# WeGoToMars/indexed_bzip2

Hardware: AMD Instinct MI355X
Metric: decompressed MB/s (whole node), 2 GiB Silesia bz2-9 (higher is better)
Workload: dtype u8

## Files before the change

### indexed_bzip2_amd/csrc/bz2_device.hip

```cpp
#include <hip/hip_runtime.h>

#include <cstdio>
#include <atomic>
#include <chrono>
#include <cstdlib>
#include <algorithm>
#include <cstring>
#include <condition_variable>
#include <memory>
#include <mutex>
#include <string>
#include <thread>
#include <vector>

#include "../../include/mi355x_bz2.h"
#include "bz2_kernels.hip.h"
#include "bz2_stage1.hip.h"
#include "bz2_hscan.hip.h"
#include "bz2_walk.hip.h"
#include "bz2_plan.hpp"
#include "bz2_scratch.hpp"
#include "bz2_lanes.hpp"
#include "bz2_ctx.hpp"

// ... 836 lines not shown
mi355x::decodeBatchBegin( mi355x_bz2_ctx* c, const uint64_t* offsets, const uint64_t* endBytes, uint32_t n )
{
    if ( c == nullptr || ( n > 0 && offsets == nullptr ) ) return MI355X_BZ2_ERR_INVALID_ARGUMENT;
    const std::scoped_lock lock( c->mutex );
    if ( c->pendingBlocks != 0 ) {
        c->lastError = "a batch is already in flight on this context: call mi355x_bz2_decode_batch_end first";
        return MI355X_BZ2_ERR_INVALID_ARGUMENT;
    }
    c->outSize = 0;
    c->lastBlocks = 0;
    if ( n == 0 ) return MI355X_BZ2_OK;
    if ( n > MI355X_BZ2_MAX_BATCH_BLOCKS ) {
        c->lastError = "more than MI355X_BZ2_MAX_BATCH_BLOCKS blocks in one batch: split it";
        return MI355X_BZ2_ERR_INVALID_ARGUMENT;
    }
    if ( c->dIn == nullptr && !c->upload ) {
        c->lastError = "no input set";
        return MI355X_BZ2_ERR_INVALID_ARGUMENT;
    }
    HIP_TRY( c, hipSetDevice( c->device ) );
    const BatchSwitches switches = readSwitches();
    const auto tBegin = std::chrono::steady_clock::now();
    int rc = ensureScratch( c, n );
    if ( rc != MI355X_BZ2_OK ) return rc;
    rc = ensureOutput( c, std::max<uint64_t>( (uint64_t)n * 900000u, c->outSizeHint ) );
    if ( rc != MI355X_BZ2_OK ) return rc;
    const auto tScratch = std::chrono::steady_clock::now();
    const uint8_t* inBase = nullptr;
    uint64_t inSize = 0;
    {
        uint64_t last = 0;
        for ( uint32_t i = 0; i < n; ++i ) last = std::max( last, offsets[i] );
        rc = awaitInput( c, last / 8 + 2400000, &inBase, &inSize );
        if ( rc != MI355X_BZ2_OK ) return rc;
    }
    const auto tInput = std::chrono::steady_clock::now();

    const bool crowd = walkChainOf( c->device ).liveContexts.load() >= 3;
    const uint32_t lanes = lanesNow( c );
    PlanOverrides knobs = switches.plan;
    if ( lanes == 1 ) knobs.noSplit = true;
    c->plan = planBatch( offsets, n, inSize, crowd, knobs );
    c->trace = switches.trace;
    const BatchPlan& plan = c->plan;
    const LaneLayout layout = layLanes( lanes, plan );
    rc = ensureLanes( c, layout );
    if ( rc != MI355X_BZ2_OK ) return rc;
    std::copy( plan.slotOf.begin(), plan.slotOf.end(), c->hSlotOf );
    std::copy( plan.offsets.begin(), plan.offsets.end(), c->hOffsets );
    std::copy( plan.order.begin(), plan.order.end(), c->hOrder );
    if ( endBytes != nullptr ) {
        for ( uint32_t i = 0; i < n; ++i ) c->hEnds[plan.slotOf[i]] = endBytes[i];
    }

    for ( auto& bits : c->launched ) bits = 0;
    if ( c->inPending ) {
        HIP_TRY( c, hipStreamWaitEvent( c->stream, c->inReady, 0 ) );
        c->inPending = false;
    }
    c->inFlight = ( inBase == c->in[0].bytes && inBase != nullptr ) ? 0 : ( ( inBase == c->in[1].bytes && inBase != nullptr ) ? 1 : -1 );
    HIP_TRY( c, hipEventRecord( c->evStep[0], c->stream ) );
    HIP_TRY( c, hipMemcpyAsync( c->dOffsets, c->hOffsets, (size_t)n * sizeof( uint64_t ), hipMemcpyHostToDevice, c->stream ) );
    HIP_TRY( c, hipMemcpyAsync( c->dOrder, c->hOrder, (size_t)n * sizeof( uint32_t ), hipMemcpyHostToDevice, c->stream ) );
    HIP_TRY( c, hipMemcpyAsync( c->dSlotOf, c->hSlotOf, (size_t)n * sizeof( uint32_t ), hipMemcpyHostToDevice, c->stream ) );
    if ( endBytes != nullptr ) {
        HIP_TRY( c, hipMemcpyAsync( c->dEnds, c->hEnds, (size_t)n * sizeof( uint64_t ), hipMemcpyHostToDevice, c->stream ) );
    }
    HIP_TRY( c, hipEventRecord( c->evStep[1], c->stream ) );
    auto streamOfLane = [&] ( int l ) { return l == layout.highLane ? c->highStream : c->lane[l]; };
    auto streamOf = [&] ( int g ) { return streamOfLane( layout.laneOf[g] ); };
    {
        bool waits[MAX_LANES]{};
        for ( int g = 0; g < plan.groups; ++g ) {
            const int l = layout.laneOf[g];
            if ( l != 0 && !waits[l] ) HIP_TRY( c, hipStreamWaitEvent( streamOfLane( l ), c->evStep[1], 0 ) );
            waits[l] = true;
        }
    }
    int lastGroupOfLane[MAX_LANES];
    for ( auto& g : lastGroupOfLane ) g = -1;

    const dim3 walkGrid( WALK_QUEUES * plan.walkWgsPerXcd );
    for ( int launch = 0; launch < plan.groups; ++launch ) {
        const int g = plan.expensive >= 0 ? ( launch == 0 ? plan.expensive : launch - 1 ) : launch;
        const uint32_t m = plan.count[g], first = plan.first[g];
        hipStream_t q = streamOf( g );
        BlockMeta* const meta = c->dMeta + first;
        HuffMeta* const hmeta = c->dHmeta + first;
        uint8_t* const sel = c->dSel + (size_t)first * SEL_STRIDE;
        uint16_t* const sym = c->dSym + (size_t)first * SYM_STRIDE;
        uint8_t* const stb = c->dStb + (size_t)first * 256;
        uint8_t* const lcol = c->dL + (size_t)first * L_STRIDE;
        uint32_t* const tab = c->dTab + (size_t)first * TAB_STRIDE;
        uint8_t* const rbuf = c->dR + (size_t)first * L_STRIDE;
        uint32_t* const segLen = c->dSegLen + (size_t)first * SEG_STRIDE;
        uint32_t* const segSucc = c->dSegSucc + (size_t)first * SEG_STRIDE;
        uint32_t* const segCont = c->dSegCont + (size_t)first * SEG_STRIDE;
        uint2* const chain = c->dChain + (size_t)first * SEG_STRIDE;
        uint32_t* const stash = c->dStash + (size_t)first * SEG_STRIDE * ( STASH_BYTES / 4 );
        const uint32_t* const order = c->dOrder + first;
        WalkPlan* const walkPlan = c->dPlan + g;
        uint32_t* const walkBlk = c->dWalkBlk + (size_t)g * ( c->capacity + 16 );
        uint32_t* const walkPre = c->dWalkPre + (size_t)g * ( c->capacity + 16 );

        {
            ScanMeta* const smeta = c->dSmeta + first;
            HuffTables* const htab = c->dHtab + first;
            uint32_t* const gpos = c->dGpos + (size_t)first * GPOS_STRIDE;
            const auto* const inWords = reinterpret_cast<const uint32_t*>( inBase );
            const uint64_t* const ends = endBytes != nullptr ? c->dEnds + first : nullptr;
            if ( plan.scanWaves[g] == 8 ) {
                TIMED_LAUNCH( c, g, q, 12, k_hscan_spec<8>, dim3( m ), dim3( 512 ), 0, q, inWords, inSize, c->dOffsets + first,
                              ends, meta, hmeta, smeta, sel, stb, htab, gpos, m, order );
            } else if ( plan.scanWaves[g] == 4 ) {
                TIMED_LAUNCH( c, g, q, 12, k_hscan_spec<4>, dim3( m ), dim3( 256 ), 0, q, inWords, inSize, c->dOffsets + first,
                              ends, meta, hmeta, smeta, sel, stb, htab, gpos, m, order );
            } else {
                TIMED_LAUNCH( c, g, q, 12, ( k_hscan<1, REGS_SCAN> ), dim3( m ), dim3( 64 ), sizeof( ScanShared<1> ), q, inWords,
                              inSize, c->dOffsets + first, ends, meta, hmeta, smeta, sel, stb, htab, gpos, m, order );
            }
#define HSYM( T ) TIMED_LAUNCH( c, g, q, 13, k_hsym<T>, dim3( ( MAX_SCAN_GROUPS + ( T ) * SYM_CHUNKS - 1 ) / ( ( T ) * SYM_CHUNKS ), m ), dim3( T ), \
                                sizeof( SymShared<T> ), q, inWords, meta, hmeta, smeta, sel, htab, gpos, sym )
            HSYM( SYM_GROUPS );
#undef HSYM
        }
#define MTF256( STRIDE, STREAM, INDEX ) \
        TIMED_LAUNCH( c, g, STREAM, INDEX, ( k_mtf<STRIDE, MTF_THREADS, REGS_MTF> ), dim3( m ), dim3( MTF_THREADS ), \
                      sizeof( MtfShared<STRIDE, MTF_THREADS> ), STREAM, meta, hmeta, sym, stb, lcol, m, order )
        const hipStream_t side = layout.sideLaneOf[g] >= 0 ? streamOfLane( layout.sideLaneOf[g] ) : q;
        if ( side != q ) {
            HIP_TRY( c, hipEventRecord( c->evFork[g], q ) );
            HIP_TRY( c, hipStreamWaitEvent( side, c->evFork[g], 0 ) );
        }
        if ( plan.mtfSmallLanes == 1024 ) {
            TIMED_LAUNCH( c, g, side, 11, ( k_mtf<MTF_SMALL_STRIDE, 1024> ), dim3( m ), dim3( 1024 ), sizeof( MtfShared<MTF_SMALL_STRIDE, 1024> ), side, meta, hmeta, sym, stb, lcol, m, order );
        } else if ( plan.mtfSmallLanes == 512 ) {
            TIMED_LAUNCH( c, g, side, 11, ( k_mtf<MTF_SMALL_STRIDE, 512> ), dim3( m ), dim3( 512 ), sizeof( MtfShared<MTF_SMALL_STRIDE, 512> ), side, meta, hmeta, sym, stb, lcol, m, order );
        } else {
            MTF256( MTF_SMALL_STRIDE, side, 11 );
        }
        if ( side != q ) HIP_TRY( c, hipEventRecord( c->evJoin[g], side ) );
        if ( plan.mtfSmallLanes > 256 ) {
            TIMED_LAUNCH( c, g, q, 1, ( k_mtf<MTF_LANE_STRIDE, 512> ), dim3( m ), dim3( 512 ), sizeof( MtfShared<MTF_LANE_STRIDE, 512> ), q, meta, hmeta, sym, stb, lcol, m, order );
        } else {
            MTF256( MTF_LANE_STRIDE, q, 1 );
        }
        if ( side != q ) HIP_TRY( c, hipStreamWaitEvent( q, c->evJoin[g], 0 ) );
#undef MTF256
        if ( plan.bwtSlices > 1 ) {
            uint32_t* const counts = c->dBwtCounts + (size_t)first * BWT_COUNTS_PER_BLOCK;
            TIMED( c, g, q, 2, hipLaunchKernelGGL( k_bwt_count, dim3( plan.bwtSlices, m ), dim3( 1024 ), 0, q, meta, lcol, counts, plan.bwtSlices );
                               hipLaunchKernelGGL( k_bwt_rank, dim3( plan.bwtSlices, m ), dim3( 1024 ), 0, q, meta, lcol, tab, counts, plan.bwtSlices ) );
        } else {
            TIMED_LAUNCH( c, g, q, 2, k_bwt_build, dim3( m ), dim3( 1024 ), 0, q, meta, lcol, tab );
        }
        TIMED_LAUNCH( c, g, q, 10, k_walk_plan, dim3( 1 ), dim3( 256 ), 0, q, meta, m, walkPlan, walkBlk, walkPre );
        {
            WalkChain& walks = walkChainOf( c->device );
            const std::scoped_lock walkLock( walks.mutex );
            if ( walks.last != nullptr ) HIP_TRY( c, hipStreamWaitEvent( q, walks.last, 0 ) );
            TIMED_LAUNCH( c, g, q, 3, k_walk, walkGrid, dim3( WALK_THREADS ), 0, q,
                          meta, tab, walkPlan, walkBlk, walkPre, segLen, segSucc, plan.walkChunk, stash, segCont );
            hipEvent_t& slot = walks.events[walks.next++ % 64];
            if ( slot == nullptr ) HIP_TRY( c, hipEventCreateWithFlags( &slot, hipEventDisableTiming ) );
            HIP_TRY( c, hipEventRecord( slot, q ) );
            walks.last = slot;
        }
        TIMED_LAUNCH( c, g, q, 4, k_link2, dim3( m ), dim3( LINK_THREADS ), sizeof( LinkShared ), q, meta, segLen, segSucc, chain );
        TIMED_LAUNCH( c, g, q, 5, k_emit, dim3( ( SEG_STRIDE + EMIT_THREADS * EMIT_TILES - 1 ) / ( EMIT_THREADS * EMIT_TILES ), m ), dim3( EMIT_THREADS ), 0, q,
                      meta, tab, chain, stash, segCont, rbuf );
        static_assert( (size_t)SEG_STRIDE * STASH_BYTES >= L_STRIDE );
        TIMED_LAUNCH( c, g, q, 6, k_replicate, dim3( m ), dim3( 256 ), 0, q, meta, rbuf, reinterpret_cast<uint8_t*>( stash ),
                      (size_t)SEG_STRIDE * STASH_BYTES );
        TIMED_LAUNCH( c, g, q, 7, k_rle<false>, dim3( m ), dim3( RLE_THREADS ), 0, q, meta, rbuf, (uint8_t*)nullptr );
        lastGroupOfLane[layout.laneOf[g]] = g;
    }
    HIP_TRY( c, hipGetLastError() );
    for ( uint32_t l = 1; l < MAX_LANES; ++l ) {
        const int g = lastGroupOfLane[l];
        if ( g < 0 ) continue;
        HIP_TRY( c, hipEventRecord( c->evGroupDone[g], streamOfLane( (int)l ) ) );
        HIP_TRY( c, hipStreamWaitEvent( c->stream, c->evGroupDone[g], 0 ) );
    }

    if ( c->outputHold != nullptr ) {
        HIP_TRY( c, hipStreamWaitEvent( c->stream, c->outputHold, 0 ) );
        c->outputHold = nullptr;
    }
    hipLaunchKernelGGL( k_offsets, dim3( 1 ), dim3( OFFSETS_THREADS ), 0, c->stream, c->dMeta, c->dSlotOf, n,
                        c->out[c->outCurrent].capacity, c->dTotals );
    rc = queueOutput( c, n, c->dTotals + 1 );
    if ( rc != MI355X_BZ2_OK ) return rc;
    HIP_TRY( c, hipMemcpyAsync( c->hTotals, c->dTotals, 2 * sizeof( uint64_t ), hipMemcpyDeviceToHost, c->stream ) );
    c->pendingBlocks = n;
    if ( switches.readerTrace ) {
        const auto ms = [] ( auto a, auto b ) { return std::chrono::duration<double, std::milli>( b - a ).count(); };
        std::fprintf( stderr, "[device] begin of %u blocks: scratch %.1f ms, input %.1f ms, plan + launches %.1f ms\n", n,
                      ms( tBegin, tScratch ), ms( tScratch, tInput ), ms( tInput, std::chrono::steady_clock::now() ) );
    }
    return MI355X_BZ2_OK;
}

int
mi355x::resultBuffer( mi355x_bz2_ctx* c, uint64_t size, uint64_t keep, uint8_t** device )
{
    if ( c == nullptr || device == nullptr ) return MI355X_BZ2_ERR_INVALID_ARGUMENT;
    const std::scoped_lock lock( c->mutex );
    HIP_TRY( c, hipSetDevice( c->device ) );
    GrowBuffer& result = c->result;
    if ( size > result.capacity || result.bytes == nullptr ) {
        HIP_TRY( c, hipStreamSynchronize( c->stream ) );
        const uint64_t cap = std::max<uint64_t>( { size, result.capacity + result.capacity / 2, uint64_t( 1 ) << 20 } );
        if ( c->dOut == result.bytes ) c->dOut = c->out[c->outCurrent].bytes;
        GrowBuffer grown;
        HIP_TRY( c, grown.grow( c, cap, cap, cap ) );
        if ( keep != 0 && result.bytes != nullptr ) {
            HIP_TRY( c, hipMemcpyAsync( grown.bytes, result.bytes, std::min( keep, result.capacity ), hipMemcpyDeviceToDevice, c->stream ) );
            HIP_TRY( c, hipStreamSynchronize( c->stream ) );
        }
        std::swap( result, grown );
        grown.putAside( c, cap );
    }
    *device = result.bytes;
    return MI355X_BZ2_OK;
}

void*&
mi355x::encoderOf( mi355x_bz2_ctx* c, void ( *release )( void* ) )
{
    c->encoderFree = release;
    return c->encoder;
}

int
mi355x::deviceOf( const mi355x_bz2_ctx* c )
{
    return c->device;
}

uint64_t
mi355x::inputCapacity( const mi355x_bz2_ctx* c )
{
    const std::scoped_lock lock( c->mutex );
    return std::max( c->in[0].capacity, c->in[1].capacity );
}

void
mi355x::setLastError( mi355x_bz2_ctx* c, const std::string& message )
{
    const std::scoped_lock lock( c->mutex );
    c->lastError = message;
}

int
mi355x::publishResult( mi355x_bz2_ctx* c, uint64_t size )
{
    if ( c == nullptr || size > c->result.capacity ) return MI355X_BZ2_ERR_INVALID_ARGUMENT;
    const std::scoped_lock lock( c->mutex );
    c->dOut = c->result.bytes;
    c->outSize = size;
    return MI355X_BZ2_OK;
}

extern "C" {

int
mi355x_bz2_decode_batch_end( mi355x_bz2_ctx* c, mi355x_bz2_block_result* results, uint64_t* totalDecoded )
{
    if ( c == nullptr ) return MI355X_BZ2_ERR_INVALID_ARGUMENT;
    const std::scoped_lock lock( c->mutex );
    if ( totalDecoded ) *totalDecoded = 0;
    const uint32_t n = c->pendingBlocks;
    if ( n == 0 ) return MI355X_BZ2_OK;
    if ( results == nullptr ) return MI355X_BZ2_ERR_INVALID_ARGUMENT;
    c->pendingBlocks = 0;
    const BatchPlan& plan = c->plan;
    int rc = MI355X_BZ2_OK;
    HIP_TRY( c, hipSetDevice( c->device ) );
    HIP_TRY( c, hipStreamSynchronize( c->stream ) );
    uint64_t total = c->hTotals[0];
    if ( c->hTotals[1] != 0 ) {
        total = 0;
        for ( uint32_t i = 0; i < n; ++i ) {
            BlockMeta& m = c->hMeta[c->hSlotOf[i]];
            m.out_off = total;
            if ( m.walk_ok ) total += m.decoded_size;
        }
        rc = ensureOutput( c, total );
        if ( rc != MI355X_BZ2_OK ) return rc;
        HIP_TRY( c, hipMemcpyAsync( c->dMeta, c->hMeta, (size_t)n * sizeof( BlockMeta ), hipMemcpyHostToDevice, c->stream ) );
        rc = queueOutput( c, n, nullptr );
        if ( rc != MI355X_BZ2_OK ) return rc;
        HIP_TRY( c, hipStreamSynchronize( c->stream ) );
    }
    c->outSizeHint = std::max( c->outSizeHint, total );

    for ( uint32_t i = 0; i < n; ++i ) {
        const BlockMeta& m = c->hMeta[c->hSlotOf[i]];
        mi355x_bz2_block_result& r = results[i];
        r.encoded_offset_bits = m.enc_off;
        r.encoded_size_bits = ( m.status == ST_OK || m.status == ST_CRC ) ? m.enc_size : 0;
        r.decoded_size = m.status == ST_OK || m.status == ST_CRC ? m.decoded_size : 0;
        r.data_offset = m.out_off;
        r.header_crc = m.header_crc;
        r.computed_crc = m.computed_crc;
        const bool loopDone = m.status == ST_OK || m.status == ST_CRC || m.status == ST_ORIGPTR_DATA;
        r.bwt_length = loopDone ? m.n : 0;
// ... 363 lines not shown
```

### indexed_bzip2_amd/csrc/bz2_kernels.hip.h

```cpp
#pragma once

#include <hip/hip_runtime.h>
#include <stdint.h>

#include "bz2_scratch.hpp"

namespace bz2gpu
{
constexpr uint32_t MAX_N = 900000;
constexpr uint32_t MIN_SEG_STRIDE = 16;
constexpr uint32_t MARK = 0x80000000u;
constexpr uint32_t LF_MASK = 0xFFFFFu;
constexpr uint32_t INVALID_OFF = 0xFFFFFFFFu;

enum Status : int32_t {
    ST_OK = 0, ST_EOF = 1, ST_BAD_MAGIC = 2, ST_RANDOMIZED = 3, ST_ORIGPTR_RANGE = 4, ST_GROUP_COUNT = 5,
    ST_SELECTOR_COUNT = 6, ST_SELECTOR_UNARY = 7, ST_CODE_LENGTH = 8, ST_HUFFMAN_LENGTHS = 9,
    ST_SELECTOR_OVERRUN = 10, ST_INVALID_CODE = 11, ST_RUN_OVERFLOW = 12, ST_DATA_OVERFLOW = 13,
    ST_ORIGPTR_DATA = 14, ST_CRC = 15
};

struct BlockMeta
{
    uint64_t enc_off;
// ... 27 lines not shown
{
    return __builtin_amdgcn_readfirstlane( v );
}

__device__ __forceinline__ uint32_t
be32( uint32_t word )
{
    return __builtin_bswap32( word );
}

__device__ __forceinline__ uint32_t
lane_id()
{
    return threadIdx.x & 63u;
}

struct BitRd
{
    const uint32_t* w;
    uint64_t nwords;
    uint64_t size_bits;
    uint32_t tail_mask;
    uint64_t buf;
    uint32_t n;
    uint64_t widx;
    uint64_t pos;
    bool eof;

    __device__ __forceinline__ uint32_t
    loadw( uint64_t i ) const
    {
        uint32_t v = 0;
        if ( i < nwords ) {
            v = sfl( be32( w[i] ) );
        }
        return v;
    }

    __device__ __forceinline__ void
    init( const uint32_t* words, uint64_t size_bytes, uint64_t bitpos )
    {
        w = words;
        nwords = ( size_bytes + 3 ) >> 2;
        size_bits = size_bytes * 8;
        const uint32_t r = (uint32_t)( size_bytes & 3 );
        tail_mask = r == 0 ? 0xFFFFFFFFu : ( 0xFFFFFFFFu << ( 32 - 8 * r ) );
        pos = bitpos;
        eof = false;
        widx = bitpos >> 5;
        const uint32_t sh = (uint32_t)( bitpos & 31 );
        const uint64_t hi = loadw( widx ), lo = loadw( widx + 1 );
        buf = ( ( hi << 32 ) | lo ) << sh;
        n = 64 - sh;
        widx += 2;
    }

    __device__ __forceinline__ void
    refill()
    {
        if ( n <= 32 ) {
            buf |= (uint64_t)loadw( widx ) << ( 32 - n );
            n += 32;
            ++widx;
        }
    }

    __device__ __forceinline__ uint32_t
    peek( uint32_t k ) const
    {
        return (uint32_t)( buf >> ( 64 - k ) );
    }

    __device__ __forceinline__ void
    skip( uint32_t k )
    {
        buf <<= k;
        n -= k;
        pos += k;
    }

    __device__ __forceinline__ uint32_t
    read( uint32_t k )
    {
        refill();
        if ( pos + k > size_bits ) {
            eof = true;
        }
        const uint32_t v = peek( k );
        skip( k );
        return v;
    }
};

__global__ __launch_bounds__( 256 ) void
k_find_magic( const uint32_t* __restrict__ words, uint64_t size_bits, uint64_t magic48,
              uint64_t* __restrict__ found, uint32_t capacity, uint32_t* __restrict__ counter )
{
    const uint64_t nStartWords = ( size_bits + 31 ) >> 5;
    const uint64_t stride = (uint64_t)gridDim.x * 256;
    for ( uint64_t w = (uint64_t)blockIdx.x * 256 + threadIdx.x; w < nStartWords; w += stride ) {
        const uint64_t hi = ( (uint64_t)be32( words[w] ) << 32 ) | be32( words[w + 1] );
        const uint64_t lo = (uint64_t)be32( words[w + 2] ) << 32;
#pragma unroll 4
        for ( uint32_t s = 0; s < 32; ++s ) {
            const uint64_t window = s == 0 ? hi : ( ( hi << s ) | ( lo >> ( 64 - s ) ) );
            if ( ( window >> 16 ) == magic48 ) {
                const uint64_t offset = w * 32 + s;
                if ( offset + 48 <= size_bits ) {
                    const uint32_t slot = atomicAdd( counter, 1u );
                    if ( slot < capacity ) found[slot] = offset;
                }
            }
        }
    }
}

__device__ __forceinline__ uint64_t
match_any( uint32_t key, int bits, bool valid )
{
    const uint64_t all = __ballot( valid );
    uint32_t lo = 0, hi = 0;
    int b = 0;
    for ( ; b + 1 < bits; b += 2 ) {
        const uint32_t minus0 = (uint32_t)__builtin_amdgcn_sbfe( (int)key, b, 1 );
        const uint32_t minus1 = (uint32_t)__builtin_amdgcn_sbfe( (int)key, b + 1, 1 );
        const uint64_t bal0 = __ballot( minus0 != 0 );
        const uint64_t bal1 = __ballot( minus1 != 0 );
        lo = lo | ( (uint32_t)bal0 ^ minus0 ) | ( (uint32_t)bal1 ^ minus1 );
        hi = hi | ( (uint32_t)( bal0 >> 32 ) ^ minus0 ) | ( (uint32_t)( bal1 >> 32 ) ^ minus1 );
    }
    if ( b < bits ) {
        const uint32_t minusBit = (uint32_t)__builtin_amdgcn_sbfe( (int)key, b, 1 );
        const uint64_t bal = __ballot( minusBit != 0 );
        lo |= (uint32_t)bal ^ minusBit;
        hi |= (uint32_t)( bal >> 32 ) ^ minusBit;
    }
    return all & ~( ( (uint64_t)hi << 32 ) | lo );
}

__device__ __forceinline__ uint64_t
match_any_runs( uint32_t key, bool valid )
{
    const uint32_t first = (uint32_t)__builtin_amdgcn_readfirstlane( (int)key );
    if ( __ballot( valid && key != first ) == 0 ) return __ballot( valid );
    return match_any( key, 8, valid );
}

__device__ __forceinline__ uint32_t
popc_below( uint64_t mask, uint32_t lane )
{
    return __popcll( mask & ( ( 1ull << lane ) - 1ull ) );
}

__global__ __launch_bounds__( 1024 ) void
k_bwt_build( const BlockMeta* __restrict__ meta,
             const uint8_t* __restrict__   l_buf,
             uint32_t* __restrict__        tab_buf )
{
    __shared__ uint32_t hist[BWT_WAVES][256];
    __shared__ uint32_t tot[256];
    const uint32_t b = blockIdx.x;
    const BlockMeta mt = meta[b];
    if ( !mt.walk_ok ) return;
    const uint32_t N = mt.n, origPtr = mt.orig_ptr, stride = mt.seg_stride;
    const uint8_t* const L = l_buf + (size_t)b * L_STRIDE;
    uint32_t* const tab = tab_buf + (size_t)b * TAB_STRIDE;
    const uint32_t tid = threadIdx.x, wave = tid >> 6, lane = tid & 63;

    uint32_t chunk = ( N + BWT_WAVES - 1 ) / BWT_WAVES;
    chunk = ( chunk + 255u ) & ~255u;
    const uint32_t begin = wave * chunk < N ? wave * chunk : N;
    const uint32_t end = begin + chunk < N ? begin + chunk : N;

    for ( uint32_t i = tid; i < BWT_WAVES * 256; i += 1024 ) ( &hist[0][0] )[i] = 0;
    __syncthreads();

    for ( uint32_t base = begin; base < end; base += 256 ) {
        const uint32_t i = base + 4 * lane;
        if ( i < end ) {
            const uint32_t v = *reinterpret_cast<const uint32_t*>( L + i );
            const uint32_t nb = end - i < 4 ? end - i : 4;
            for ( uint32_t k = 0; k < nb; ++k ) atomicAdd( &hist[wave][( v >> ( 8 * k ) ) & 0xFF], 1u );
        }
    }
    __syncthreads();
    if ( tid < 256 ) {
        uint32_t run = 0;
        for ( int w = 0; w < BWT_WAVES; ++w ) {
            const uint32_t t = hist[w][tid];
            hist[w][tid] = run;
            run += t;
        }
        tot[tid] = run;
    }
    __syncthreads();
    if ( tid < 64 ) {
        uint32_t v0 = tot[4 * tid], v1 = tot[4 * tid + 1], v2 = tot[4 * tid + 2], v3 = tot[4 * tid + 3];
        const uint32_t s = v0 + v1 + v2 + v3;
        uint32_t incl = s;
        for ( int d = 1; d < 64; d <<= 1 ) {
            const uint32_t o = __shfl_up( incl, d );
            if ( (int)tid >= d ) incl += o;
        }
        uint32_t excl = incl - s;
        tot[4 * tid] = excl; excl += v0;
        tot[4 * tid + 1] = excl; excl += v1;
        tot[4 * tid + 2] = excl; excl += v2;
        tot[4 * tid + 3] = excl;
    }
    __syncthreads();
    if ( tid < 256 ) {
        const uint32_t c = tot[tid];
        for ( int w = 0; w < BWT_WAVES; ++w ) hist[w][tid] += c;
    }
    __syncthreads();

    uint32_t rem = ( begin + lane ) % stride;
    const uint32_t remStep = 64u % stride;
    for ( uint32_t base4 = begin; base4 < end; base4 += 256 ) {
        uint32_t keys[4];
#pragma unroll
        for ( uint32_t u = 0; u < 4; ++u ) keys[u] = L[base4 + 64 * u + lane];
#pragma unroll
        for ( uint32_t u = 0; u < 4; ++u ) {
            const uint32_t i = base4 + 64 * u + lane;
            const bool valid = i < end;
            const uint32_t key = valid ? keys[u] : 0u;
            const uint64_t same = match_any_runs( key, valid );
            const uint32_t rank = popc_below( same, lane );
            uint32_t basePos = 0;
            if ( valid ) basePos = hist[wave][key];
            if ( valid ) {
                const uint32_t lf = basePos + rank;
                const bool mark = ( rem == 0 ) || ( i == origPtr );
                tab[i] = ( lf << 8 ) | key | ( mark ? MARK : 0u );
                if ( rank == 0 ) hist[wave][key] = basePos + (uint32_t)__popcll( same );
            }
            rem += remStep;
            if ( rem >= stride ) rem -= stride;
        }
    }
}

__device__ __forceinline__ void
bwt_chunk_range( uint32_t N, uint32_t slices, uint32_t slice, uint32_t wave, uint32_t& begin, uint32_t& end )
{
    uint32_t chunk = ( N + slices * BWT_WAVES - 1 ) / ( slices * BWT_WAVES );
    chunk = ( chunk + 255u ) & ~255u;
    const uint32_t index = slice * BWT_WAVES + wave;
    begin = index * chunk < N ? index * chunk : N;
    end = begin + chunk < N ? begin + chunk : N;
}

__global__ __launch_bounds__( 1024 ) void
k_bwt_count( const BlockMeta* __restrict__ meta,
             const uint8_t* __restrict__   l_buf,
             uint32_t* __restrict__        counts,
             uint32_t                      slices )
{
    __shared__ uint32_t hist[BWT_WAVES][256];
    const uint32_t b = blockIdx.y, slice = blockIdx.x;
    const BlockMeta mt = meta[b];
    if ( !mt.walk_ok ) return;
    const uint8_t* const L = l_buf + (size_t)b * L_STRIDE;
    const uint32_t tid = threadIdx.x, wave = tid >> 6, lane = tid & 63;
    uint32_t begin, end;
    bwt_chunk_range( mt.n, slices, slice, wave, begin, end );
    for ( uint32_t i = tid; i < BWT_WAVES * 256; i += 1024 ) ( &hist[0][0] )[i] = 0;
    __syncthreads();
    for ( uint32_t base = begin; base < end; base += 256 ) {
        const uint32_t i = base + 4 * lane;
        if ( i < end ) {
            const uint32_t v = *reinterpret_cast<const uint32_t*>( L + i );
            const uint32_t nb = end - i < 4 ? end - i : 4;
            for ( uint32_t k = 0; k < nb; ++k ) atomicAdd( &hist[wave][( v >> ( 8 * k ) ) & 0xFF], 1u );
        }
    }
    __syncthreads();
    uint32_t* const out = counts + (size_t)b * BWT_COUNTS_PER_BLOCK + (size_t)slice * BWT_WAVES * 256;
    for ( uint32_t i = tid; i < BWT_WAVES * 256; i += 1024 ) out[i] = ( &hist[0][0] )[i];
}

__global__ __launch_bounds__( 1024 ) void
k_bwt_rank( const BlockMeta* __restrict__ meta,
            const uint8_t* __restrict__   l_buf,
            uint32_t* __restrict__        tab_buf,
            const uint32_t* __restrict__  counts,
            uint32_t                      slices )
{
    __shared__ uint32_t hist[BWT_WAVES][256];
    __shared__ uint32_t tot[256];
    const uint32_t b = blockIdx.y, slice = blockIdx.x;
    const BlockMeta mt = meta[b];
    if ( !mt.walk_ok ) return;
    const uint32_t N = mt.n, origPtr = mt.orig_ptr, stride = mt.seg_stride;
    const uint8_t* const L = l_buf + (size_t)b * L_STRIDE;
    uint32_t* const tab = tab_buf + (size_t)b * TAB_STRIDE;
    const uint32_t tid = threadIdx.x, wave = tid >> 6, lane = tid & 63;
    if ( tid < 256 ) {
        const uint32_t* const of = counts + (size_t)b * BWT_COUNTS_PER_BLOCK + tid;
        uint32_t run = 0;
        for ( uint32_t c = 0; c < slices * BWT_WAVES; ++c ) {
            const uint32_t t = of[(size_t)c * 256];
            if ( c / BWT_WAVES == slice ) hist[c % BWT_WAVES][tid] = run;
            run += t;
        }
        tot[tid] = run;
    }
    __syncthreads();
    if ( tid < 64 ) {
        uint32_t v0 = tot[4 * tid], v1 = tot[4 * tid + 1], v2 = tot[4 * tid + 2], v3 = tot[4 * tid + 3];
        const uint32_t s4 = v0 + v1 + v2 + v3;
        uint32_t incl = s4;
        for ( int d = 1; d < 64; d <<= 1 ) {
            const uint32_t o = __shfl_up( incl, d );
            if ( (int)tid >= d ) incl += o;
        }
        uint32_t excl = incl - s4;
        tot[4 * tid] = excl; excl += v0;
        tot[4 * tid + 1] = excl; excl += v1;
        tot[4 * tid + 2] = excl; excl += v2;
        tot[4 * tid + 3] = excl;
    }
    __syncthreads();
    if ( tid < 256 ) {
        const uint32_t c = tot[tid];
        for ( int w = 0; w < BWT_WAVES; ++w ) hist[w][tid] += c;
    }
    __syncthreads();

    uint32_t begin, end;
    bwt_chunk_range( N, slices, slice, wave, begin, end );
    uint32_t rem = ( begin + lane ) % stride;
    const uint32_t remStep = 64u % stride;
    for ( uint32_t base4 = begin; base4 < end; base4 += 256 ) {
        uint32_t keys[4];
#pragma unroll
        for ( uint32_t u = 0; u < 4; ++u ) keys[u] = L[base4 + 64 * u + lane];
#pragma unroll
        for ( uint32_t u = 0; u < 4; ++u ) {
            const uint32_t i = base4 + 64 * u + lane;
            const bool valid = i < end;
            const uint32_t key = valid ? keys[u] : 0u;
            const uint64_t same = match_any_runs( key, valid );
            const uint32_t rank = popc_below( same, lane );
            uint32_t basePos = 0;
            if ( valid ) basePos = hist[wave][key];
            if ( valid ) {
                const uint32_t lf = basePos + rank;
                const bool mark = ( rem == 0 ) || ( i == origPtr );
                tab[i] = ( lf << 8 ) | key | ( mark ? MARK : 0u );
                if ( rank == 0 ) hist[wave][key] = basePos + (uint32_t)__popcll( same );
            }
            rem += remStep;
            if ( rem >= stride ) rem -= stride;
        }
    }
}

__global__ __launch_bounds__( 256 ) void
k_replicate( const BlockMeta* __restrict__ meta,
             uint8_t*                      r_buf,
             uint8_t*                      tmp_buf,
             size_t                        tmp_stride )
{
    const uint32_t b = blockIdx.x;
    const BlockMeta mt = meta[b];
    if ( !mt.walk_ok || mt.cycle_len >= mt.n || mt.cycle_len == 0 ) return;
    const uint32_t N = mt.n, c = mt.cycle_len;
    uint8_t* const R = r_buf + (size_t)b * L_STRIDE;
    const uint32_t r = N % c;
    if ( r == 0 ) {
        for ( uint32_t k = c + threadIdx.x; k < N; k += 256 ) {
            R[N - 1 - k] = R[N - 1 - ( k % c )];
        }
        return;
    }
    uint8_t* const Y = tmp_buf + (size_t)b * tmp_stride;
    for ( uint32_t k = threadIdx.x; k < c; k += 256 ) Y[k] = R[N - 1 - k];
    __syncthreads();
    for ( uint32_t k = threadIdx.x; k < N; k += 256 ) {
        R[N - 1 - k] = Y[( k % c + c - r ) % c];
    }
}

constexpr uint32_t RLE_THREADS = 512;
constexpr uint32_t RLE_BYTES_PER_THREAD = 32;
constexpr uint32_t RLE_TILE = RLE_THREADS * RLE_BYTES_PER_THREAD;
constexpr uint32_t FN_IDENTITY = 0 | ( 1 << 3 ) | ( 2 << 6 ) | ( 3 << 9 ) | ( 4 << 12 );

__device__ __forceinline__ uint32_t
fn_apply( uint32_t f, uint32_t k )
// ... 405 lines not shown
```

### indexed_bzip2_amd/csrc/bz2_walk.hip.h

```cpp
#pragma once

#include "bz2_kernels.hip.h"

namespace bz2gpu
{
constexpr uint32_t WALK_THREADS = 256;
constexpr uint32_t WALK_QUEUES = 8;
constexpr uint32_t EMIT_THREADS = 256;
constexpr uint32_t EMIT_TILES = 4;
constexpr uint32_t EMIT_STAGE = 16384;

struct WalkPlan
{
    uint32_t q_begin[WALK_QUEUES + 1];
    uint32_t q_total[WALK_QUEUES];
    uint32_t ctr[WALK_QUEUES];
    uint32_t pad[15];
};

__global__ __launch_bounds__( 256 ) void
k_walk_plan( const BlockMeta* __restrict__ meta, uint32_t n, WalkPlan* plan, uint32_t* blk, uint32_t* pre )
{
    __shared__ uint32_t begin[WALK_QUEUES + 1];
    const uint32_t t = threadIdx.x;
    if ( t == 0 ) {
        uint32_t acc = 0;
        for ( uint32_t q = 0; q < WALK_QUEUES; ++q ) {
            begin[q] = acc;
            acc += q < n ? ( n - q + WALK_QUEUES - 1 ) / WALK_QUEUES : 0;
        }
        begin[WALK_QUEUES] = acc;
    }
    __syncthreads();
    if ( t <= WALK_QUEUES ) plan->q_begin[t] = begin[t];
    if ( t < WALK_QUEUES ) {
        uint32_t idx = begin[t], acc = 0;
        for ( uint32_t i = t; i < n; i += WALK_QUEUES ) {
            blk[idx] = i;
            pre[idx] = acc;
            acc += meta[i].walk_ok ? meta[i].nseg : 0u;
            ++idx;
        }
        plan->q_total[t] = acc;
        plan->ctr[t] = 0;
    }
}

constexpr uint32_t LINK_THREADS = 256;
constexpr uint32_t LINK_SPLIT = 128;
constexpr uint32_t LINK_MAX_SUB = KMAX / LINK_SPLIT + 2;

struct alignas( 16 ) LinkShared
{
    uint16_t ssucc[SEG_STRIDE];
    uint32_t subLen[LINK_MAX_SUB];
    uint16_t subNext[LINK_MAX_SUB];
    uint32_t subOff[LINK_MAX_SUB];
    uint32_t subCnt[LINK_MAX_SUB];
    uint32_t subRank[LINK_MAX_SUB];
};

__device__ __forceinline__ void
link_block( BlockMeta*                   meta,
            const uint32_t* __restrict__ seg_len,
            const uint32_t* __restrict__ seg_succ,
            uint2* __restrict__          chain,
            uint16_t* __restrict__       ssucc,
            uint32_t* __restrict__       subLen,
            uint16_t* __restrict__       subNext,
            uint32_t* __restrict__       subOff,
            uint32_t* __restrict__       subCnt,
            uint32_t* __restrict__       subRank )
{
    const uint32_t b = blockIdx.x;
    const BlockMeta mt = meta[b];
    if ( !mt.walk_ok ) return;
    const uint32_t nseg = mt.nseg, N = mt.n, stride = mt.seg_stride, origPtr = mt.orig_ptr;
    const uint32_t k0 = ( N + stride - 1 ) / stride;
    const size_t base = (size_t)b * SEG_STRIDE;
    const uint32_t first = ( origPtr % stride != 0 ) ? k0 : origPtr / stride;
    const uint32_t tid = threadIdx.x;

    for ( uint32_t j = tid; j < nseg; j += LINK_THREADS ) {
        const uint32_t s = seg_succ[base + j];
        ssucc[j] = (uint16_t)( s < nseg ? s : 0xFFFFu );
    }
    const uint32_t nSplit = ( nseg + LINK_SPLIT - 1 ) / LINK_SPLIT;
    const bool firstExtra = first % LINK_SPLIT != 0;
    const uint32_t nSub = nSplit + ( firstExtra ? 1u : 0u );
    const auto splitterOf = [&] ( uint32_t seg ) -> uint32_t {
        if ( seg == first && firstExtra ) return nSplit;
        return seg % LINK_SPLIT == 0 ? seg / LINK_SPLIT : 0xFFFFu;
    };
    for ( uint32_t s = tid; s < LINK_MAX_SUB; s += LINK_THREADS ) subOff[s] = INVALID_OFF;
    __syncthreads();

    constexpr uint32_t AHEAD = 8;
    for ( uint32_t s = tid; s < nSub; s += LINK_THREADS ) {
        uint32_t cur = s < nSplit ? s * LINK_SPLIT : first;
        uint32_t sum = 0, steps = 0, nextSub = 0xFFFFu;
        bool more = true;
        while ( more ) {
            uint32_t nodes[AHEAD];
            uint32_t m = 0;
#pragma unroll
            for ( uint32_t k = 0; k < AHEAD; ++k ) {
                nodes[k] = cur;
                if ( more ) {
                    m = k + 1;
                    cur = ssucc[cur];
                    ++steps;
                    if ( cur == 0xFFFFu || steps > nseg ) {
                        more = false;
                    } else {
                        nextSub = splitterOf( cur );
                        more = nextSub == 0xFFFFu;
                    }
                }
            }
#pragma unroll
            for ( uint32_t k = 0; k < AHEAD; ++k ) {
                if ( k < m ) sum += seg_len[base + nodes[k]];
            }
        }
        subLen[s] = sum;
        subCnt[s] = steps;
        subNext[s] = (uint16_t)nextSub;
    }
    __syncthreads();

    if ( tid == 0 ) {
        const uint32_t start = firstExtra ? nSplit : first / LINK_SPLIT;
        uint32_t s = start, off = 0, visited = 0, rank = 0;
        bool ok = true;
        do {
            subOff[s] = off;
            subRank[s] = rank;
            off += subLen[s];
            rank += subCnt[s];
            s = subNext[s];
            ++visited;
            if ( s == 0xFFFFu || visited > nSub || off > N ) { ok = false; break; }
        } while ( s != start );
        meta[b].cycle_len = off;
        meta[b].nchain = rank;
        if ( !ok || off == 0 ) {
            meta[b].status = ST_CRC;
            meta[b].walk_ok = 0;
        }
    }
    __syncthreads();

    for ( uint32_t s = tid; s < nSub; s += LINK_THREADS ) {
        uint32_t off = subOff[s];
        if ( off == INVALID_OFF ) continue;
        uint32_t cur = s < nSplit ? s * LINK_SPLIT : first;
        uint32_t steps = 0;
        uint32_t rank = subRank[s];
        bool more = true;
        while ( more ) {
            uint32_t nodes[AHEAD], lens[AHEAD];
            uint32_t m = 0;
#pragma unroll
            for ( uint32_t k = 0; k < AHEAD; ++k ) {
                nodes[k] = cur;
                if ( more ) {
                    m = k + 1;
                    cur = ssucc[cur];
                    ++steps;
                    more = !( cur == 0xFFFFu || steps > nseg || splitterOf( cur ) != 0xFFFFu );
                }
            }
#pragma unroll
            for ( uint32_t k = 0; k < AHEAD; ++k ) lens[k] = k < m ? seg_len[base + nodes[k]] : 0u;
#pragma unroll
            for ( uint32_t k = 0; k < AHEAD; ++k ) {
                if ( k < m ) {
                    const uint32_t len = lens[k];
                    chain[base + rank] = make_uint2( off | ( nodes[k] << 20 ), len | ( ( nodes[k] >> 12 ) << 20 ) );
                    ++rank;
                    off += len;
                }
            }
        }
    }
}

__global__ __launch_bounds__( LINK_THREADS ) void
k_link2( BlockMeta*                   meta,
         const uint32_t* __restrict__ seg_len,
         const uint32_t* __restrict__ seg_succ,
         uint2* __restrict__          chain )
{
    extern __shared__ __attribute__( ( aligned( 16 ) ) ) uint8_t ldsAtLaunch[];
    auto& shared = *reinterpret_cast<LinkShared*>( ldsAtLaunch );
    link_block( meta, seg_len, seg_succ, chain, shared.ssucc, shared.subLen, shared.subNext, shared.subOff,
                shared.subCnt, shared.subRank );
}

__global__ __launch_bounds__( WALK_THREADS ) void
k_walk( const BlockMeta* __restrict__ meta,
         const uint32_t* __restrict__  tab_buf,
         WalkPlan*                     plan,
         const uint32_t* __restrict__  blk,
         const uint32_t* __restrict__  pre,
         uint32_t*                     seg_len,
         uint32_t*                     seg_succ,
         uint32_t                      chunk,
         uint32_t*                     stash,
         uint32_t*                     seg_cont )
{
    __shared__ uint32_t sBase, sNext, sK0;
    const uint32_t tid = threadIdx.x;
    const uint32_t lane = tid & 63u;
    uint32_t xcc;
    asm volatile( "s_getreg_b32 %0, hwreg(HW_REG_XCC_ID)" : "=s"( xcc ) );
    xcc &= WALK_QUEUES - 1;

    for ( uint32_t attempt = 0; attempt < WALK_QUEUES; ++attempt ) {
        const uint32_t q = ( xcc + attempt ) & ( WALK_QUEUES - 1 );
        const uint32_t qb = plan->q_begin[q], qe = plan->q_begin[q + 1];
        const uint32_t total = plan->q_total[q];
        if ( total == 0 ) continue;
        for ( ;; ) {
            __syncthreads();
            if ( tid == 0 ) {
                const uint32_t base = atomicAdd( &plan->ctr[q], chunk );
                sBase = base;
                uint32_t lo = qb, hi = qe;
                while ( hi - lo > 1 ) {
                    const uint32_t mid = ( lo + hi ) >> 1;
                    if ( pre[mid] <= base ) lo = mid; else hi = mid;
                }
                sK0 = lo;
            }
            __syncthreads();
            uint32_t base = sBase;
            if ( base >= total ) break;
            const uint32_t claimEnd = total - base < chunk ? total : base + chunk;
            uint32_t k = sK0;
            while ( base < claimEnd ) {
                while ( k + 1 < qe && base >= pre[k + 1] ) ++k;
                const uint32_t runEnd = ( k + 1 < qe && pre[k + 1] < claimEnd ) ? pre[k + 1] : claimEnd;
                const uint32_t cnt = runEnd - base;
                const uint32_t b = blk[k];
                const uint32_t j0 = base - pre[k];
                const uint32_t N = meta[b].n, stride = meta[b].seg_stride, origPtr = meta[b].orig_ptr;
                const uint32_t k0 = ( N + stride - 1 ) / stride;
                const uint32_t* const tab = tab_buf + (size_t)b * TAB_STRIDE;
                const size_t segBase = (size_t)b * SEG_STRIDE;
                uint32_t* const stashOfBlock = stash + segBase * ( STASH_BYTES / 4 );
                __syncthreads();
                if ( tid == 0 ) sNext = WALK_THREADS;
                __syncthreads();

                uint32_t my = tid;
                bool idle = true;
                uint32_t j = 0, p = 0, e = 0, len = 0, piece = 0;
                for ( ;; ) {
                    if ( idle && my < cnt ) {
                        j = j0 + my;
                        p = j < k0 ? j * stride : origPtr;
                        e = tab[p];
                        len = 0;
                        piece = 0;
                        idle = false;
                    }
                    if ( __ballot( !idle ) == 0 ) break;
                    if ( !idle ) {
                        uint32_t w[4] = { 0, 0, 0, 0 };
                        bool done = false;
                        if ( piece == STASH_BYTES / 16 ) __builtin_nontemporal_store( p, seg_cont + segBase + j );
#pragma unroll
                        for ( uint32_t i = 0; i < 16; i += 4 ) {
                            if ( !done ) {
#pragma unroll
                                for ( uint32_t s4 = i; s4 < i + 4; ++s4 ) {
                                    const uint32_t live = done ? 0u : 1u;
                                    w[s4 >> 2] |= done ? 0u : ( e & 0xFFu ) << ( 8 * ( s4 & 3u ) );
                                    len += live;
                                    p = done ? p : ( e >> 8 ) & LF_MASK;
                                    e = tab[p];
                                    done = ( e & MARK ) || len >= N;
                                }
                            }
                        }
                        if ( piece < STASH_BYTES / 16 ) {
                            uint32_t* const out = stashOfBlock + (size_t)j * ( STASH_BYTES / 4 ) + 4 * piece;
                            __builtin_nontemporal_store( w[0], out );
                            __builtin_nontemporal_store( w[1], out + 1 );
                            __builtin_nontemporal_store( w[2], out + 2 );
                            __builtin_nontemporal_store( w[3], out + 3 );
                        }
                        ++piece;
                        if ( done ) {
                            __builtin_nontemporal_store( len, seg_len + segBase + j );
                            const bool isOrig = ( p == origPtr ) && ( origPtr % stride != 0 );
                            __builtin_nontemporal_store( ( e & MARK ) ? ( isOrig ? k0 : p / stride ) : 0xFFFFFFFFu, seg_succ + segBase + j );
                            idle = true;
                        }
                    }
                    {
                        const uint64_t asking = __ballot( idle );
                        if ( asking != 0 ) {
                            uint32_t first = 0;
                            if ( lane == (uint32_t)__builtin_ctzll( asking ) ) first = atomicAdd( &sNext, (uint32_t)__popcll( asking ) );
                            first = (uint32_t)__builtin_amdgcn_readlane( (int)first, __builtin_ctzll( asking ) );
                            const uint32_t rank = __builtin_amdgcn_mbcnt_hi( (uint32_t)( asking >> 32 ), __builtin_amdgcn_mbcnt_lo( (uint32_t)asking, 0 ) );
                            if ( idle ) my = first < cnt ? first + rank : cnt;
                        }
                    }
                }
                base = runEnd;
            }
        }
    }
}
__global__ __launch_bounds__( EMIT_THREADS ) void
k_emit( const BlockMeta* __restrict__ meta,
        const uint32_t* __restrict__  tab_buf,
        const uint2* __restrict__     chain,
        const uint32_t* __restrict__  stash,
        const uint32_t* __restrict__  seg_cont,
        uint8_t* __restrict__         r_buf )
{
    constexpr uint32_t STASH = STASH_BYTES, STAGE = EMIT_STAGE;
    constexpr uint32_t FIRST = 2;
    constexpr uint32_t MORE = STASH / 16 - FIRST;
    __shared__ __attribute__( ( aligned( 16 ) ) ) uint8_t image[STAGE + 16];
    __shared__ uint32_t sLow, sTop;
    __shared__ uint32_t segAddr[EMIT_THREADS], segLen[EMIT_THREADS], segId[EMIT_THREADS];
    __shared__ uint16_t later[EMIT_THREADS * MORE];
    __shared__ uint32_t waveSum[EMIT_THREADS / 64];
    const uint32_t b = blockIdx.y;
    const BlockMeta mt = meta[b];
    if ( !mt.walk_ok ) return;
    const uint32_t t = threadIdx.x;
    const uint32_t N = mt.n;
    for ( uint32_t tile = 0; tile < EMIT_TILES; ++tile ) {
    const uint32_t r0 = ( blockIdx.x * EMIT_TILES + tile ) * EMIT_THREADS;
    if ( r0 >= mt.nchain ) return;
    const uint32_t count = mt.nchain - r0 < EMIT_THREADS ? mt.nchain - r0 : EMIT_THREADS;
    const size_t base = (size_t)b * SEG_STRIDE;
    uint8_t* const R = r_buf + (size_t)b * L_STRIDE;
    const uint32_t* const tab = tab_buf + (size_t)b * TAB_STRIDE;
    const uint32_t* const stashOfBlock = stash + base * ( STASH_BYTES / 4 );

    uint2 rec = make_uint2( 0, 0 );
    if ( t < count ) rec = chain[base + r0 + t];
// ... 90 lines not shown
```

Before: 34150.

## Rewrite BWT build as single-wave per-lane counting and cache segment lengths in link

The BWT table build moves from a 1024-thread block with per-wave histograms and ballot-based rank matching to one 64-lane wave per block. Each lane owns a contiguous slice, counts into a private LDS column, and then a DPP wave scan produces prefix offsets. Loads are 16-byte vectors prefetched several units ahead, and mark bits are folded in with byte permutes. Separately, the link kernel doubles its threads, halves the split size, caches segment lengths as 16-bit values in LDS, and simplifies the traversal loops. The tradeoff is far fewer threads per BWT block, which depends on many blocks being resident to fill the GPU, plus more LDS per link block.

```diff
diff --git a/indexed_bzip2_amd/csrc/bz2_device.hip b/indexed_bzip2_amd/csrc/bz2_device.hip
--- a/indexed_bzip2_amd/csrc/bz2_device.hip
+++ b/indexed_bzip2_amd/csrc/bz2_device.hip
@@ -1012,7 +1012,7 @@
             TIMED( c, g, q, 2, hipLaunchKernelGGL( k_bwt_count, dim3( plan.bwtSlices, m ), dim3( 1024 ), 0, q, meta, lcol, counts, plan.bwtSlices );
                                hipLaunchKernelGGL( k_bwt_rank, dim3( plan.bwtSlices, m ), dim3( 1024 ), 0, q, meta, lcol, tab, counts, plan.bwtSlices ) );
         } else {
-            TIMED_LAUNCH( c, g, q, 2, k_bwt_build, dim3( m ), dim3( 1024 ), 0, q, meta, lcol, tab );
+            TIMED_LAUNCH( c, g, q, 2, k_bwt_build, dim3( m ), dim3( 64 ), 0, q, meta, lcol, tab );
         }
         TIMED_LAUNCH( c, g, q, 10, k_walk_plan, dim3( 1 ), dim3( 256 ), 0, q, meta, m, walkPlan, walkBlk, walkPre );
         {
diff --git a/indexed_bzip2_amd/csrc/bz2_kernels.hip.h b/indexed_bzip2_amd/csrc/bz2_kernels.hip.h
--- a/indexed_bzip2_amd/csrc/bz2_kernels.hip.h
+++ b/indexed_bzip2_amd/csrc/bz2_kernels.hip.h
@@ -203,92 +203,148 @@
     return __popcll( mask & ( ( 1ull << lane ) - 1ull ) );
 }
 
-__global__ __launch_bounds__( 1024 ) void
+__device__ __forceinline__ uint32_t
+wave_inclusive_sum( uint32_t v )
+{
+#define BZ2_DPP_ADD( CTRL, ROWS ) v += (uint32_t)__builtin_amdgcn_update_dpp( 0, (int)v, CTRL, ROWS, 0xF, true )
+    BZ2_DPP_ADD( 0x111, 0xF );
+    BZ2_DPP_ADD( 0x112, 0xF );
+    BZ2_DPP_ADD( 0x114, 0xF );
+    BZ2_DPP_ADD( 0x118, 0xF );
+    BZ2_DPP_ADD( 0x142, 0xA );
+    BZ2_DPP_ADD( 0x143, 0xC );
+#undef BZ2_DPP_ADD
+    return v;
+}
+
+constexpr uint32_t BWT_UNIT = 16;
+constexpr uint32_t BWT_AHEAD = 4;
+
+__device__ __forceinline__ void
+bwt_settle( uint4 ( &q )[BWT_AHEAD] )
+{
+#pragma unroll
+    for ( uint32_t k = 0; k < BWT_AHEAD; ++k ) asm volatile( "" : "+v"( q[k].x ), "+v"( q[k].y ), "+v"( q[k].z ), "+v"( q[k].w ) );
+    __builtin_amdgcn_s_waitcnt( 0x0F70 );
+}
+
+__device__ __forceinline__ uint32_t*
+bwt_counter( uint8_t* column, uint32_t value )
+{
+    return reinterpret_cast<uint32_t*>( column + (uint32_t)( value << 8 ) );
+}
+
+__device__ __forceinline__ void
+bwt_count_unit( uint8_t* column, const uint4& bytes )
+{
+    const uint32_t w[4] = { bytes.x, bytes.y, bytes.z, bytes.w };
+#pragma unroll
+    for ( uint32_t e = 0; e < BWT_UNIT; ++e ) atomicAdd( bwt_counter( column, ( w[e / 4] >> ( 8 * ( e % 4 ) ) ) & 0xFFu ), 1u );
+}
+
+__device__ __forceinline__ void
+bwt_rank_unit( uint8_t* column, const uint4& bytes, uint32_t* __restrict__ tab, uint32_t i, uint32_t& nextMark, uint32_t stride,
+               uint32_t origPtr )
+{
+    uint64_t maskLo = 0, maskHi = 0;
+    const auto maskByte = [&maskLo, &maskHi] ( uint32_t d ) {
+        maskLo |= d < 8u ? 0x80ull << ( 8u * d ) : 0ull;
+        maskHi |= d - 8u < 8u ? 0x80ull << ( 8u * ( d - 8u ) ) : 0ull;
+    };
+    maskByte( nextMark - i );
+    if ( nextMark - i < BWT_UNIT ) nextMark += stride;
+    if ( __ballot( origPtr - i < BWT_UNIT ) != 0 ) maskByte( origPtr - i );
+    const uint32_t w[4] = { bytes.x, bytes.y, bytes.z, bytes.w };
+    const uint32_t mk[4] = { (uint32_t)maskLo, (uint32_t)( maskLo >> 32 ), (uint32_t)maskHi, (uint32_t)( maskHi >> 32 ) };
+    uint32_t x[BWT_UNIT], lf[BWT_UNIT];
+#pragma unroll
+    for ( uint32_t e = 0; e < BWT_UNIT; ++e ) {
+        x[e] = __builtin_amdgcn_perm( mk[e / 4], w[e / 4], ( ( 4u + e % 4 ) << 24 ) | 0x0C0C00u | ( e % 4 ) );
+        lf[e] = atomicAdd( bwt_counter( column, x[e] ), 1u );
+    }
+#pragma unroll
+    for ( uint32_t e = 0; e < BWT_UNIT; e += 4 ) {
+        *reinterpret_cast<uint4*>( tab + i + e ) = make_uint4( ( lf[e] << 8 ) | x[e], ( lf[e + 1] << 8 ) | x[e + 1],
+                                                               ( lf[e + 2] << 8 ) | x[e + 2], ( lf[e + 3] << 8 ) | x[e + 3] );
+    }
+}
+
+__global__ __launch_bounds__( 64 ) void
 k_bwt_build( const BlockMeta* __restrict__ meta,
              const uint8_t* __restrict__   l_buf,
              uint32_t* __restrict__        tab_buf )
 {
-    __shared__ uint32_t hist[BWT_WAVES][256];
-    __shared__ uint32_t tot[256];
+    __shared__ uint32_t cnt[256 * 64];
     const uint32_t b = blockIdx.x;
     const BlockMeta mt = meta[b];
     if ( !mt.walk_ok ) return;
     const uint32_t N = mt.n, origPtr = mt.orig_ptr, stride = mt.seg_stride;
     const uint8_t* const L = l_buf + (size_t)b * L_STRIDE;
     uint32_t* const tab = tab_buf + (size_t)b * TAB_STRIDE;
-    const uint32_t tid = threadIdx.x, wave = tid >> 6, lane = tid & 63;
-
-    uint32_t chunk = ( N + BWT_WAVES - 1 ) / BWT_WAVES;
-    chunk = ( chunk + 255u ) & ~255u;
-    const uint32_t begin = wave * chunk < N ? wave * chunk : N;
-    const uint32_t end = begin + chunk < N ? begin + chunk : N;
-
-    for ( uint32_t i = tid; i < BWT_WAVES * 256; i += 1024 ) ( &hist[0][0] )[i] = 0;
-    __syncthreads();
-
-    for ( uint32_t base = begin; base < end; base += 256 ) {
-        const uint32_t i = base + 4 * lane;
-        if ( i < end ) {
-            const uint32_t v = *reinterpret_cast<const uint32_t*>( L + i );
-            const uint32_t nb = end - i < 4 ? end - i : 4;
-            for ( uint32_t k = 0; k < nb; ++k ) atomicAdd( &hist[wave][( v >> ( 8 * k ) ) & 0xFF], 1u );
-        }
-    }
-    __syncthreads();
-    if ( tid < 256 ) {
-        uint32_t run = 0;
-        for ( int w = 0; w < BWT_WAVES; ++w ) {
-            const uint32_t t = hist[w][tid];
-            hist[w][tid] = run;
-            run += t;
-        }
-        tot[tid] = run;
-    }
-    __syncthreads();
-    if ( tid < 64 ) {
-        uint32_t v0 = tot[4 * tid], v1 = tot[4 * tid + 1], v2 = tot[4 * tid + 2], v3 = tot[4 * tid + 3];
-        const uint32_t s = v0 + v1 + v2 + v3;
-        uint32_t incl = s;
-        for ( int d = 1; d < 64; d <<= 1 ) {
-            const uint32_t o = __shfl_up( incl, d );
-            if ( (int)tid >= d ) incl += o;
-        }
-        uint32_t excl = incl - s;
-        tot[4 * tid] = excl; excl += v0;
-        tot[4 * tid + 1] = excl; excl += v1;
-        tot[4 * tid + 2] = excl; excl += v2;
-        tot[4 * tid + 3] = excl;
-    }
-    __syncthreads();
-    if ( tid < 256 ) {
-        const uint32_t c = tot[tid];
-        for ( int w = 0; w < BWT_WAVES; ++w ) hist[w][tid] += c;
-    }
-    __syncthreads();
-
-    uint32_t rem = ( begin + lane ) % stride;
-    const uint32_t remStep = 64u % stride;
-    for ( uint32_t base4 = begin; base4 < end; base4 += 256 ) {
-        uint32_t keys[4];
-#pragma unroll
-        for ( uint32_t u = 0; u < 4; ++u ) keys[u] = L[base4 + 64 * u + lane];
-#pragma unroll
-        for ( uint32_t u = 0; u < 4; ++u ) {
-            const uint32_t i = base4 + 64 * u + lane;
-            const bool valid = i < end;
-            const uint32_t key = valid ? keys[u] : 0u;
-            const uint64_t same = match_any_runs( key, valid );
-            const uint32_t rank = popc_below( same, lane );
-            uint32_t basePos = 0;
-            if ( valid ) basePos = hist[wave][key];
-            if ( valid ) {
-                const uint32_t lf = basePos + rank;
-                const bool mark = ( rem == 0 ) || ( i == origPtr );
-                tab[i] = ( lf << 8 ) | key | ( mark ? MARK : 0u );
-                if ( rank == 0 ) hist[wave][key] = basePos + (uint32_t)__popcll( same );
-            }
-            rem += remStep;
-            if ( rem >= stride ) rem -= stride;
+    const uint32_t lane = threadIdx.x;
+    uint8_t* const column = reinterpret_cast<uint8_t*>( cnt ) + 4 * lane;
+
+    static_assert( ( ( MAX_N + 63 ) / 64 + BWT_UNIT - 1 ) / BWT_UNIT * BWT_UNIT * 64 <= L_STRIDE && BWT_AHEAD * BWT_UNIT <= 256 );
+    const uint32_t units = ( ( N + 63u ) / 64u + BWT_UNIT - 1u ) / BWT_UNIT;
+    const uint32_t unitsAhead = units & ~( BWT_AHEAD - 1u );
+    const uint32_t lo = lane * units * BWT_UNIT;
+    const uint4* const mine = reinterpret_cast<const uint4*>( L + lo );
+
+#pragma unroll 8
+    for ( uint32_t v = 0; v < 256; ++v ) cnt[v * 64 + lane] = 0;
+
+    {
+        const uint32_t tail = N & ~( BWT_UNIT - 1u );
+        const uint32_t end = lo + units * BWT_UNIT;
+        const uint32_t wholeEnd = end < tail ? end : tail;
+        uint4 q[BWT_AHEAD];
+#pragma unroll
+        for ( uint32_t k = 0; k < BWT_AHEAD; ++k ) q[k] = mine[k];
+        bwt_settle( q );
+        for ( uint32_t u0 = 0; u0 < unitsAhead; u0 += BWT_AHEAD ) {
+#pragma unroll
+            for ( uint32_t k = 0; k < BWT_AHEAD; ++k ) {
+                if ( lo + ( u0 + k + 1 ) * BWT_UNIT <= wholeEnd ) bwt_count_unit( column, q[k] );
+                q[k] = mine[u0 + k + BWT_AHEAD];
+            }
+        }
+#pragma unroll
+        for ( uint32_t k = 0; k < BWT_AHEAD - 1; ++k ) {
+            if ( unitsAhead + k < units && lo + ( unitsAhead + k + 1 ) * BWT_UNIT <= wholeEnd ) bwt_count_unit( column, q[k] );
+        }
+        if ( tail >= lo && tail < end ) {
+            for ( uint32_t p = tail; p < N; ++p ) atomicAdd( bwt_counter( column, L[p] ), 1u );
+        }
+    }
+
+    {
+        uint32_t carry = 0;
+#pragma unroll 4
+        for ( uint32_t v = 0; v < 256; ++v ) {
+            const uint32_t x = cnt[v * 64 + lane];
+            const uint32_t incl = wave_inclusive_sum( x );
+            cnt[v * 64 + lane] = carry + incl - x;
+            carry += (uint32_t)__builtin_amdgcn_readlane( (int)incl, 63 );
+        }
+    }
+
+    {
+        static_assert( TAB_STRIDE >= L_STRIDE );
+        uint32_t nextMark = ( lo + stride - 1u ) / stride * stride;
+        uint4 q[BWT_AHEAD];
+#pragma unroll
+        for ( uint32_t k = 0; k < BWT_AHEAD; ++k ) q[k] = mine[k];
+        bwt_settle( q );
+        for ( uint32_t u0 = 0; u0 < unitsAhead; u0 += BWT_AHEAD ) {
+#pragma unroll
+            for ( uint32_t k = 0; k < BWT_AHEAD; ++k ) {
+                bwt_rank_unit( column, q[k], tab, lo + ( u0 + k ) * BWT_UNIT, nextMark, stride, origPtr );
+                q[k] = mine[u0 + k + BWT_AHEAD];
+            }
+        }
+#pragma unroll
+        for ( uint32_t k = 0; k < BWT_AHEAD - 1; ++k ) {
+            if ( unitsAhead + k < units ) bwt_rank_unit( column, q[k], tab, lo + ( unitsAhead + k ) * BWT_UNIT, nextMark, stride, origPtr );
         }
     }
 }
diff --git a/indexed_bzip2_amd/csrc/bz2_walk.hip.h b/indexed_bzip2_amd/csrc/bz2_walk.hip.h
--- a/indexed_bzip2_amd/csrc/bz2_walk.hip.h
+++ b/indexed_bzip2_amd/csrc/bz2_walk.hip.h
@@ -46,13 +46,15 @@
     }
 }
 
-constexpr uint32_t LINK_THREADS = 256;
-constexpr uint32_t LINK_SPLIT = 128;
+constexpr uint32_t LINK_THREADS = 512;
+constexpr uint32_t LINK_SPLIT = 64;
 constexpr uint32_t LINK_MAX_SUB = KMAX / LINK_SPLIT + 2;
+constexpr uint32_t LINK_LONG = 0xFFFFu;
 
 struct alignas( 16 ) LinkShared
 {
     uint16_t ssucc[SEG_STRIDE];
+    uint16_t slen[SEG_STRIDE];
     uint32_t subLen[LINK_MAX_SUB];
     uint16_t subNext[LINK_MAX_SUB];
     uint32_t subOff[LINK_MAX_SUB];
@@ -66,6 +68,7 @@
             const uint32_t* __restrict__ seg_succ,
             uint2* __restrict__          chain,
             uint16_t* __restrict__       ssucc,
+            uint16_t* __restrict__       slen,
             uint32_t* __restrict__       subLen,
             uint16_t* __restrict__       subNext,
             uint32_t* __restrict__       subOff,
@@ -83,8 +86,14 @@
 
     for ( uint32_t j = tid; j < nseg; j += LINK_THREADS ) {
         const uint32_t s = seg_succ[base + j];
+        const uint32_t len = seg_len[base + j];
         ssucc[j] = (uint16_t)( s < nseg ? s : 0xFFFFu );
-    }
+        slen[j] = (uint16_t)( len < LINK_LONG ? len : LINK_LONG );
+    }
+    const auto lengthOf = [&] ( uint32_t seg ) -> uint32_t {
+        const uint32_t len = slen[seg];
+        return len != LINK_LONG ? len : seg_len[base + seg];
+    };
     const uint32_t nSplit = ( nseg + LINK_SPLIT - 1 ) / LINK_SPLIT;
     const bool firstExtra = first % LINK_SPLIT != 0;
     const uint32_t nSub = nSplit + ( firstExtra ? 1u : 0u );
@@ -95,33 +104,16 @@
     for ( uint32_t s = tid; s < LINK_MAX_SUB; s += LINK_THREADS ) subOff[s] = INVALID_OFF;
     __syncthreads();
 
-    constexpr uint32_t AHEAD = 8;
     for ( uint32_t s = tid; s < nSub; s += LINK_THREADS ) {
         uint32_t cur = s < nSplit ? s * LINK_SPLIT : first;
         uint32_t sum = 0, steps = 0, nextSub = 0xFFFFu;
-        bool more = true;
-        while ( more ) {
-            uint32_t nodes[AHEAD];
-            uint32_t m = 0;
-#pragma unroll
-            for ( uint32_t k = 0; k < AHEAD; ++k ) {
-                nodes[k] = cur;
-                if ( more ) {
-                    m = k + 1;
-                    cur = ssucc[cur];
-                    ++steps;
-                    if ( cur == 0xFFFFu || steps > nseg ) {
-                        more = false;
-                    } else {
-                        nextSub = splitterOf( cur );
-                        more = nextSub == 0xFFFFu;
-                    }
-                }
-            }
-#pragma unroll
-            for ( uint32_t k = 0; k < AHEAD; ++k ) {
-                if ( k < m ) sum += seg_len[base + nodes[k]];
-            }
+        for ( ;; ) {
+            sum += lengthOf( cur );
+            cur = ssucc[cur];
+            ++steps;
+            if ( cur == 0xFFFFu || steps > nseg ) break;
+            nextSub = splitterOf( cur );
+            if ( nextSub != 0xFFFFu ) break;
         }
         subLen[s] = sum;
         subCnt[s] = steps;
@@ -157,31 +149,14 @@
         uint32_t cur = s < nSplit ? s * LINK_SPLIT : first;
         uint32_t steps = 0;
         uint32_t rank = subRank[s];
-        bool more = true;
-        while ( more ) {
-            uint32_t nodes[AHEAD], lens[AHEAD];
-            uint32_t m = 0;
-#pragma unroll
-            for ( uint32_t k = 0; k < AHEAD; ++k ) {
-                nodes[k] = cur;
-                if ( more ) {
-                    m = k + 1;
-                    cur = ssucc[cur];
-                    ++steps;
-                    more = !( cur == 0xFFFFu || steps > nseg || splitterOf( cur ) != 0xFFFFu );
-                }
-            }
-#pragma unroll
-            for ( uint32_t k = 0; k < AHEAD; ++k ) lens[k] = k < m ? seg_len[base + nodes[k]] : 0u;
-#pragma unroll
-            for ( uint32_t k = 0; k < AHEAD; ++k ) {
-                if ( k < m ) {
-                    const uint32_t len = lens[k];
-                    chain[base + rank] = make_uint2( off | ( nodes[k] << 20 ), len | ( ( nodes[k] >> 12 ) << 20 ) );
-                    ++rank;
-                    off += len;
-                }
-            }
+        for ( ;; ) {
+            const uint32_t len = lengthOf( cur );
+            chain[base + rank] = make_uint2( off | ( cur << 20 ), len | ( ( cur >> 12 ) << 20 ) );
+            ++rank;
+            off += len;
+            cur = ssucc[cur];
+            ++steps;
+            if ( cur == 0xFFFFu || steps > nseg || splitterOf( cur ) != 0xFFFFu ) break;
         }
     }
 }
@@ -194,7 +169,7 @@
 {
     extern __shared__ __attribute__( ( aligned( 16 ) ) ) uint8_t ldsAtLaunch[];
     auto& shared = *reinterpret_cast<LinkShared*>( ldsAtLaunch );
-    link_block( meta, seg_len, seg_succ, chain, shared.ssucc, shared.subLen, shared.subNext, shared.subOff,
+    link_block( meta, seg_len, seg_succ, chain, shared.ssucc, shared.slen, shared.subLen, shared.subNext, shared.subOff,
                 shared.subCnt, shared.subRank );
 }
 
```

Result: slower. 33070 (-3.2%).
